# Lumina-Group/libzkp

Measured on AMD Instinct MI355X. Metric: proofs/sec (whole node) + ms/proof p50, 4096-proof mixed batch (range / equality / membership / improvement) per MI355X, higher is better.
Workload: dtype u32/u64 integer limbs (10x25.5-bit GF(2^255-19), BN254 Fq on 9x29-bit limbs in the MSM loops and 10x26-bit elsewhere, 8x32-bit Fr and scalars mod l, 2x64-bit f128)

## Files before the change

### libzkp_amd/csrc/bp_steps.h

```cpp
#pragma once
#include "fe25519.h"
#include "sc25519.h"
#include "ge25519.h"
#include "keccak.h"

namespace zkp {

constexpr uint32_t BP_N = 64;
constexpr uint32_t BASE_B = 0, BASE_BB = 1, BASE_G = 2, BASE_H = 66, NBASE = 130;
constexpr uint32_t WBITS = 10, NWIN = 26, NENT = 512, DIGW = 13, NWIN_U64 = 7, NIELS_W = 30, SUBTAB_W = NENT * NIELS_W;
constexpr uint32_t TAPE_SLOTS = 132;
constexpr uint32_t P1_V = 0, P1_A = 2, P1_NSLOTS = 260;
constexpr uint32_t P2_NSLOTS = 4;
constexpr uint32_t PR_NSLOTS = 130;
ZKP_HD constexpr uint32_t p1_s(uint32_t n) { return 3 + 2 * n; }
ZKP_HD constexpr uint32_t tape_slots(uint32_t n) { return 2 * n + 4; }
ZKP_HD constexpr uint32_t rp_bytes(uint32_t lg) { return 32 * (9 + 2 * lg); }
constexpr uint32_t GE_W = 40;
enum { SC_Y = 0, SC_Z, SC_X, SC_W, SC_U, SC_UINV, SC_T0, SC_T1, SC_T2, SC_NUM };
enum { KIND_RANGE_MIN = 0, KIND_RANGE_MAX, KIND_THRESHOLD, KIND_CONSISTENCY, KIND_BULLETPROOF, KIND_NUM };

struct BpView {
    uint32_t M;
    uint32_t n, lg;
// ... 102 lines not shown
    n = ge_niels_select(d < 0, ge_niels_neg(n), n);
    return ge_madd(acc, n);
}
ZKP_HD inline void st_ge(uint32_t* p, uint32_t idx, uint32_t row, uint32_t rows, const ge& g) {
    uint32_t* q = p + (size_t)idx * GE_W * rows + row;
    ZKP_UNROLL for (int k = 0; k < 10; k++) {
        q[(size_t)k * rows] = g.X.v[k]; q[(size_t)(10 + k) * rows] = g.Y.v[k];
        q[(size_t)(20 + k) * rows] = g.Z.v[k]; q[(size_t)(30 + k) * rows] = g.T.v[k];
    }
}
ZKP_HD inline ge ld_ge(const uint32_t* p, uint32_t idx, uint32_t row, uint32_t rows) {
    ge g; const uint32_t* q = p + (size_t)idx * GE_W * rows + row;
    ZKP_UNROLL for (int k = 0; k < 10; k++) {
        g.X.v[k] = q[(size_t)k * rows]; g.Y.v[k] = q[(size_t)(10 + k) * rows];
        g.Z.v[k] = q[(size_t)(20 + k) * rows]; g.T.v[k] = q[(size_t)(30 + k) * rows];
    }
    return g;
}
struct MsmView {
    uint32_t rows, nslots, nchunks;
    const uint32_t* table;
    const uint32_t* digits;
    const uint16_t* slot_base;
    const uint16_t* slot_scalar;
    const uint8_t* slot_nwin;
    const uint16_t* chunk_begin;
    const uint16_t* chunk_win0;
    const uint16_t* chunk_nwin;
    uint32_t* partial;
    const uint32_t* acc_init;
    uint32_t nwin = 0, nent = 0, digw = 0;
    uint32_t slot_ent = 0, uneven = 0;
    const uint32_t* steps = nullptr; const uint32_t* chunk_step0 = nullptr;
};
ZKP_HD inline void msm_chunk_ref(const MsmView& m, uint32_t chunk, uint32_t row) {
    ge acc = ge_identity();
    uint32_t s = m.chunk_begin[chunk], w = m.chunk_win0[chunk];
    for (uint32_t left = m.chunk_nwin[chunk]; left > 0; left--) {
        const uint32_t srow = m.slot_scalar ? m.slot_scalar[s] : s;
        const int32_t d = ld_digit(m.digits, srow, w, row, m.rows);
        if (d != 0) acc = msm_accumulate_digit(acc, d, m.table + ((size_t)m.slot_base[s] * NWIN + w) * SUBTAB_W);
        if (++w == m.slot_nwin[s]) { s++; w = 0; }
    }
    st_ge(m.partial, chunk, row, m.rows, acc);
}
struct ReduceView {
    uint32_t rows, ntargets;
    const uint32_t* partial;
    const uint16_t* target_chunk_begin;
    uint32_t* enc;
    const uint64_t* out_off;
    uint8_t* out;
    const uint32_t* corr;
};
ZKP_HD inline void reduce_encode_thread(const ReduceView& r, uint32_t target, uint32_t row) {
    const uint32_t c0 = r.target_chunk_begin[target], c1 = r.target_chunk_begin[target + 1];
    ge acc = ld_ge(r.partial, c0, row, r.rows);
    for (uint32_t c = c0 + 1; c < c1; c++) acc = ge_add(acc, ld_ge(r.partial, c, row, r.rows));
    sc e; ge_ristretto_encode(e.v, acc);
    st_sc(r.enc, target, row, r.rows, e);
    if (r.out_off != nullptr && target == 0) put_bytes(r.out + r.out_off[row], e.v, 8);
}

ZKP_HD inline void strobe_save(const BpView& V, uint32_t job, const Strobe& s) {
    for (int i = 0; i < 50; i++) V.tstate[(size_t)i * V.M + job] = s.base[i * s.stride];
    V.tstate[(size_t)50 * V.M + job] = s.pos; V.tstate[(size_t)51 * V.M + job] = s.pos_begin;
}
ZKP_HD inline void strobe_load(const BpView& V, uint32_t job, Strobe& s) {
    for (int i = 0; i < 50; i++) s.base[i * s.stride] = V.tstate[(size_t)i * V.M + job];
    s.pos = V.tstate[(size_t)50 * V.M + job]; s.pos_begin = V.tstate[(size_t)51 * V.M + job];
}
ZKP_HD inline sc merlin_challenge_scalar(Strobe& s, const char* label, uint32_t label_len) {
    uint32_t w[16]; merlin_challenge_words(s, label, label_len, w, 16);
    return sc_from_wide(w);
}
ZKP_HD inline void merlin_append_scalar(Strobe& s, const char* label, uint32_t label_len, const sc& raw) { merlin_append_words(s, label, label_len, raw.v, 8); }

ZKP_HD inline void step_transcript1(const BpView& V, uint32_t job, Strobe& s) {
    const uint32_t M = V.M;
    switch (V.kind[job]) {
        case KIND_RANGE_MIN: merlin_init(s, "libzkp_range_min", 16); break;
        case KIND_RANGE_MAX: merlin_init(s, "libzkp_range_max", 16); break;
        case KIND_THRESHOLD: merlin_init(s, "libzkp_threshold", 16); break;
        case KIND_CONSISTENCY: merlin_init(s, "libzkp_consistency", 18); break;
        default: merlin_init(s, "libzkp_bulletproof", 18); break;
    }
    merlin_append_bytes(s, "dom-sep", 7, "rangeproof v1", 13);
    merlin_append_u64(s, "n", 1, V.n);
    merlin_append_u64(s, "m", 1, 1);
    const sc Ve = ld_sc(V.enc, 0, job, M), Ae = ld_sc(V.enc, 1, job, M), Se = ld_sc(V.enc, 2, job, M);
    merlin_append_words(s, "V", 1, Ve.v, 8);
    merlin_append_words(s, "A", 1, Ae.v, 8);
    merlin_append_words(s, "S", 1, Se.v, 8);
    const sc y = merlin_challenge_scalar(s, "y", 1);
    const sc z = merlin_challenge_scalar(s, "z", 1);
    strobe_save(V, job, s);
    st_sc(V.scal, SC_Y, job, M, y);
    st_sc(V.scal, SC_Z, job, M, z);
    const sc yinv = sc_invert(y);
    for (uint32_t h = 0; h < 2; h++) {
        const sc base = h ? yinv : y;
        sc p = sc_one();
        for (uint32_t b = 0; b < 8; b++) { st_sc(V.ypq, 16 * h + b, job, M, p); p = sc_mul(p, base); }
        sc q = sc_one();
        for (uint32_t a = 0; a < 8; a++) { st_sc(V.ypq, 16 * h + 8 + a, job, M, q); q = sc_mul(q, p); }
    }
    uint8_t* pr = V.out + V.proof_off[job];
    put_bytes(pr, Ae.v, 8); put_bytes(pr + 32, Se.v, 8);
    put_bytes(V.out + V.commit_off[job], Ve.v, 8);
// ... 199 lines not shown
```

### libzkp_amd/csrc/g16_impl.inc

```

namespace {

struct G16Key {
    bool loaded = false;
    uint32_t n_inst = 0, n_wit = 0, nv = 0, n_rows = 0, m = 0, logm = 0;
    G16Circuit C{};
    std::vector<void*> allocs;
    uint32_t *table_g1 = nullptr, *table_g2 = nullptr;
    G16Radix rx = g16_radix(G16_WBITS_DEFAULT);
    int shared_tables = -1;
    uint64_t table_bytes = 0;
    struct Chunking { DevLayout lay; const uint32_t* corr = nullptr; const uint16_t* scal = nullptr; };
    std::vector<SlotList> targets_g1, targets_g2;
    std::vector<uint16_t> hscal_g1, hscal_g2;
    std::map<uint64_t, Chunking> lays_g1, lays_g2;
    uint64_t win_g1 = 0, win_g2 = 0;
    const uint32_t *init_g1 = nullptr, *init_g2 = nullptr;
    G16Vk vk{}; bool vk_ready = false;
    uint64_t vk_table_bytes = 0;
    bool verifier_only() const { return vk_ready && !loaded; }
    const uint32_t *vm_kconst = nullptr, *vm_lines = nullptr;
};
struct G16Run {
    void* buf = nullptr; size_t cap = 0; hipStream_t side = nullptr, side2 = nullptr; hipEvent_t ev[4] = {nullptr, nullptr, nullptr, nullptr};
// ... 37 lines not shown
g2_aff host_g2_generator() {
    static const char* dec[4] = {"10857046999023057135944570762232829481370756359578518086990519993285655852781",
                                 "11559732032986387107991004021392285783925812861821192530917403151452391805634",
                                 "8495653923123431417604973247489272438418190587263600148770280649306958101930",
                                 "4082367875863433681332203403145435568316851327593401208105741076214120093531"};
    fq c[4];
    for (int k = 0; k < 4; k++) {
        fq acc = fq_zero(); const fq ten = fq_from_u64(10);
        for (const char* q = dec[k]; *q; q++) acc = fq_add(fq_mul(acc, ten), fq_from_u64((uint64_t)(*q - '0')));
        c[k] = acc;
    }
    return g2_aff{fq2{c[0], c[1]}, fq2{c[2], c[3]}};
}
g1_aff host_g1_generator() { return g1_aff{fq_from_u64(1), fq_from_u64(2)}; }
struct MsmOffsets { g1_jac o1; g2_jac o2; bool ready = false; };
MsmOffsets g_off;
std::once_flag g_off_once;
void compute_offsets();
void ensure_offsets() { std::call_once(g_off_once, compute_offsets); }
void compute_offsets() {
    uint8_t h[32]; const char* tag = "libzkp-amd msm offset"; sha256_host(h, (const uint8_t*)tag, strlen(tag));
    uint32_t k[8]; memcpy(k, h, 32); k[7] &= 0x0fffffffu;
    g_off.o1 = jac_mul_raw(jac_from_aff(host_g1_generator()), k);
    g_off.o2 = jac_mul_raw(jac_from_aff(host_g2_generator()), k);
    g_off.ready = true;
}
template <class J> J host_neg_multiple(const J& o, uint32_t k) {
    J acc = o; for (uint32_t i = 1; i < k; i++) acc = jac_add(acc, o);
    return jac_neg(acc);
}
template <class J> void append_words(std::vector<uint32_t>& v, const J& p) { const uint32_t* w = reinterpret_cast<const uint32_t*>(&p); for (size_t i = 0; i < sizeof(J) / 4; i++) v.push_back(w[i]); }
int upload_offset_point(G16Key& K, bool g2, const uint32_t** d_init) {
    ensure_offsets();
    std::vector<uint32_t> init;
    if (!g2) append_words(init, g_off.o1); else append_words(init, g_off.o2);
    return dev_upload(K, d_init, init);
}
uint32_t choose_chunks(uint64_t windows, uint32_t ntargets, uint32_t rows, uint32_t resident, uint32_t tb) {
    const uint32_t groups = (rows + tb - 1) / tb;
    uint32_t hi = (uint32_t)(windows / 8); if (hi > 2048) hi = 2048; if (hi < ntargets) hi = ntargets;
    uint32_t best = ntargets; double best_cost = 1e300;
    for (uint32_t c = ntargets; c <= hi; c++) {
        const double rounds = std::ceil((double)c * groups / resident);
        const double cost = rounds * (std::ceil((double)windows / c) + 2.5) + 0.25 * c / 8.0;
        if (cost < best_cost) { best_cost = cost; best = c; }
    }
    return best;
}
enum { G16_PART_ALL = 0, G16_PART_AB = 1, G16_PART_C = 2 };
int get_chunking(G16Key& K, bool g2, int part, uint32_t rows, const G16Key::Chunking** out) {
    const uint32_t resident = (uint32_t)dev().num_cu * g16_msm_blocks_per_cu(g2);
    const auto& all = g2 ? K.targets_g2 : K.targets_g1;
    std::vector<SlotList> targets;
    if (part == G16_PART_ALL) targets = all;
    else if (part == G16_PART_AB) targets.assign(all.begin(), all.begin() + 2);
    else targets.assign(all.begin() + 2, all.end());
    uint64_t windows = 0; for (auto& t : targets) for (auto& sl : t) windows += sl.second;
    uint32_t c = choose_chunks(windows, (uint32_t)targets.size(), rows, resident, g16_msm_rows_per_block(g2));
    if (g_budget_request >= 10000) c = g_budget_request - 10000;
    auto& cache = g2 ? K.lays_g2 : K.lays_g1;
    const uint64_t key = (uint64_t)part << 32 | c;
    auto it = cache.find(key);
    if (it == cache.end()) {
        const MsmLayout L = make_layout_even(targets, c);
        G16Key::Chunking ch; int rc;
        const auto& hs = g2 ? K.hscal_g2 : K.hscal_g1;
        std::vector<uint16_t> scal; for (uint16_t b : L.slot_base) scal.push_back(hs[b]);
        const GatherShape shape{K.rx.nent, K.rx.slot_ent, K.rx.uneven ? 1u : 0u, K.rx.digw};
        if ((rc = upload_layout(ch.lay, L, &shape, scal.data()))) return rc;
        std::vector<uint32_t> corr;
        for (uint32_t t = 0; t < L.ntargets(); t++) {
            const uint32_t k = L.target_chunk_begin[t + 1] - L.target_chunk_begin[t];
            if (!g2) append_words(corr, host_neg_multiple(g_off.o1, k)); else append_words(corr, host_neg_multiple(g_off.o2, k));
        }
        if ((rc = dev_upload(K, &ch.corr, corr))) return rc;
        if ((rc = dev_upload(K, &ch.scal, scal))) return rc;
        it = cache.emplace(key, ch).first;
    }
    *out = &it->second;
    return 0;
}


uint64_t key_table_bytes(size_t n1, size_t n2, uint32_t wbits, bool uneven = false) {
    const G16Radix rx = g16_radix(wbits, uneven);
    return ((uint64_t)n1 * g16_table_entry_words(false, true) + (uint64_t)n2 * g16_table_entry_words(true, true)) * 4ull * rx.slot_ent;
}
int choose_radix(size_t n1, size_t n2, uint32_t* wbits_out, bool* uneven_out) {
    *uneven_out = false;
    const int forced = env_int("ZKP_HIP_G16_WBITS", 0);
    if (forced) {
        if (forced < (int)G16_WBITS_MIN || forced > (int)G16_WBITS_MAX) return fail(ZKP_HIP_E_ARGUMENT, "ZKP_HIP_G16_WBITS must be 8..15");
        *wbits_out = (uint32_t)forced; *uneven_out = forced == 14 && env_int("ZKP_HIP_G16_UNEVEN", 1) != 0; return 0;
    }
    size_t free_b = 0, total_b = 0;
    HIP_TRY(hipMemGetInfo(&free_b, &total_b));
    const int budget_mb = env_int("ZKP_HIP_G16_TABLE_BUDGET_MB", 0);
    const uint64_t reserve = 8ull << 30;
    const uint64_t fits = free_b > reserve ? (uint64_t)((free_b - reserve) * 0.45) : 0;
    uint64_t budget = budget_mb > 0 ? (uint64_t)budget_mb << 20 : fits;
    uint32_t first = G16_WBITS_KNEE;
    if (budget_mb > 0) {
        first = G16_WBITS_DEFAULT;
        if (G16_WBITS_DEFAULT == 14 && env_int("ZKP_HIP_G16_UNEVEN", 1) != 0 && key_table_bytes(n1, n2, 14, true) <= budget) { *wbits_out = 14; *uneven_out = true; return 0; }
    }
    for (uint32_t w = first; w >= G16_WBITS_MIN; w--)
        if (key_table_bytes(n1, n2, w) <= budget) { *wbits_out = w; return 0; }
    char msg[256];
    snprintf(msg, sizeof msg, "not enough device memory for the proving key's window tables: %llu MB at the smallest radix (2^%u), budget %llu MB (%llu MB free)",
             (unsigned long long)(key_table_bytes(n1, n2, G16_WBITS_MIN) >> 20), G16_WBITS_MIN, (unsigned long long)(budget >> 20), (unsigned long long)(free_b >> 20));
    return fail(ZKP_HIP_E_RUNTIME, msg);
}
struct SharedTables { int hip_dev, kind; uint8_t digest[32]; uint32_t wbits; uint32_t *g1, *g2; int refs; };
struct TableRegistry { std::mutex mu; std::vector<SharedTables> v; std::map<int, std::unique_ptr<std::mutex>> build_mu; };
TableRegistry& table_registry() { static TableRegistry* r = new TableRegistry(); return *r; }
void release_shared_tables(G16Key& K) {
    if (K.shared_tables < 0) return;
    TableRegistry& R = table_registry();
    std::lock_guard<std::mutex> lk(R.mu);
    SharedTables& e = R.v[(size_t)K.shared_tables];
    if (--e.refs == 0) { (void)hipFree(e.g1); (void)hipFree(e.g2); e.g1 = e.g2 = nullptr; }
    K.shared_tables = -1; K.table_g1 = K.table_g2 = nullptr;
}

template <uint32_t AW, class Pt>
int build_tables(G16Key& K, const std::vector<Pt>& bases, uint32_t** table, bool msm_form, const G16Radix& rx, bool owned = true) {
    std::vector<uint32_t> flat; flat.reserve(bases.size() * AW);
    for (auto& b : bases) { const uint32_t* w = reinterpret_cast<const uint32_t*>(&b); for (uint32_t k = 0; k < AW; k++) flat.push_back(w[k]); }
    uint32_t* d_bases = nullptr; int rc;
    if ((rc = dev_upload(K, &d_bases, flat))) return rc;
    const size_t words = bases.size() * (size_t)rx.slot_ent * g16_table_entry_words(AW == 40, msm_form);
    uint32_t* tab = nullptr;
    if (hipMalloc(&tab, words * 4 + 64) != hipSuccess) {
        (void)hipGetLastError();
        char msg[200]; snprintf(msg, sizeof msg, "out of device memory allocating %llu MB of key tables (radix 2^%u)", (unsigned long long)((words * 4) >> 20), rx.wbits);
        return fail(ZKP_HIP_E_RUNTIME, msg);
    }
    if (owned) K.allocs.push_back(tab);
    g16_launch_build_table(AW == 40, d_bases, (uint32_t)bases.size(), tab, dev().stream, msm_form, rx);
    HIP_TRY(hipGetLastError());
    HIP_TRY(hipStreamSynchronize(dev().stream));
    *table = tab;
    return 0;
}

void release_key(G16Key& K) {
    (void)hipDeviceSynchronize();
    release_shared_tables(K);
    for (void* p : K.allocs) (void)hipFree(p);
    for (auto& e : K.lays_g1) free_layout(e.second.lay);
    for (auto& e : K.lays_g2) free_layout(e.second.lay);
    K = G16Key();
}
int load_key_body(int kind, const uint8_t* pk, uint64_t len);
int no_proving_key(const G16Key& K) {
    return fail(ZKP_HIP_E_ARGUMENT, K.verifier_only() ? "only a verifying key is loaded for this circuit: proving needs the proving key (zkp_hip_groth16_load_key)"
                                                      : "no proving key loaded for this circuit (zkp_hip_groth16_load_key)");
}
int load_key_locked(int kind, const uint8_t* pk, uint64_t len) {
    if (kind != G16_EQUALITY && kind != G16_MEMBERSHIP) return fail(ZKP_HIP_E_ARGUMENT, "unknown circuit kind");
    G16Key& K = g16s().key[kind];
    if (K.loaded || K.shared_tables >= 0 || !K.allocs.empty()) release_key(K);
    int rc;
    try { rc = load_key_body(kind, pk, len); }
    catch (...) { release_key(K); throw; }
    if (rc) { const std::string keep = t_err; release_key(K); t_err = keep; }
// ... 2 lines not shown
int install_verifying_key(G16Key& K, const G16VkBlob& B) {
    int rc;
    K.vk_ready = false;
    std::vector<uint32_t> icw; for (auto& e : B.abc) append_words(icw, e.p);
    append_words(icw, B.alpha_g1.p);
    const uint32_t* d_ic = nullptr;
    if ((rc = dev_upload(K, &d_ic, icw))) return rc;
    std::vector<g1_aff> ic_pts; for (auto& e : B.abc) ic_pts.push_back(e.p);
    ic_pts.push_back(B.alpha_g1.p);
    uint32_t* d_ic_tab = nullptr;
    const G16Radix vrx = g16_radix(G16V_WBITS);
    if ((rc = build_tables<20>(K, ic_pts, &d_ic_tab, false, vrx))) return rc;
    K.vk_table_bytes = (uint64_t)ic_pts.size() * vrx.slot_ent * g16_table_entry_words(false, false) * 4ull;
    K.vk.gamma = B.gamma_g2.p; K.vk.delta = B.delta_g2.p; K.vk.beta = B.beta_g2.p; K.vk.n_ic = (uint32_t)B.abc.size(); K.vk.ic = d_ic; K.vk.ic_table = d_ic_tab;
    K.vk.ml_alpha_beta = miller_loop(B.beta_g2.p, aff_neg(B.alpha_g1.p));
    std::vector<uint32_t> kc(6 * 20), lines;
    g16_vm_key_constants(B.beta_g2.p, aff_neg(B.alpha_g1.p), B.gamma_g2.p, B.delta_g2.p, kc.data(), lines);
    if ((rc = dev_upload(K, &K.vm_kconst, kc)) || (rc = dev_upload(K, &K.vm_lines, lines))) return rc;
    K.vk_ready = true;
    return 0;
}
int ensure_mimc_dev() {
    if (g16s().mimc_dev) return 0;
    ensure_mimc_constants();
    std::vector<uint32_t> mc; for (auto& c : g_mimc_host) put_fr(mc, c);
    HIP_TRY(hipMalloc(&g16s().mimc_dev, mc.size() * 4)); HIP_TRY(hipMemcpy(g16s().mimc_dev, mc.data(), mc.size() * 4, hipMemcpyHostToDevice));
    return 0;
}
int load_key_body(int kind, const uint8_t* pk, uint64_t len) {
    G16Key& K = g16s().key[kind];
    const HostR1CS cs = kind == G16_EQUALITY ? build_equality_r1cs() : build_membership_r1cs();
    int rc;
    KeyReader R{pk, len};
    G16VkBlob B;
    const int format = g16_read_key_prefix(R, B);
    if (format == G16_BLOB_MALFORMED)
        return fail(ZKP_HIP_E_ARGUMENT, "malformed proving key or verifying key (expected ark-serialize uncompressed ProvingKey<Bn254>, or its VerifyingKey<Bn254> alone)");
    if (format == G16_BLOB_VERIFYING_KEY) {
        if (const char* why = g16_check_verifying_key(B, cs.n_inst)) return fail(ZKP_HIP_E_ARGUMENT, why);
        return install_verifying_key(K, B);
    }
    if ((rc = upload_circuit(K, cs)) || (rc = ensure_mimc_dev())) return rc;
    const G1Pt &alpha_g1 = B.alpha_g1; const G2Pt &beta_g2 = B.beta_g2, &delta_g2 = B.delta_g2;
    const std::vector<G1Pt>& abc = B.abc;
    G1Pt beta_g1, delta_g1;
    std::vector<G1Pt> aq, b1q, hq, lq; std::vector<G2Pt> b2q;
    if (parse_g1(R, beta_g1.inf, beta_g1.p) || parse_g1(R, delta_g1.inf, delta_g1.p) ||
        parse_vec_g1(R, aq) || parse_vec_g1(R, b1q) || parse_vec_g2(R, b2q) || parse_vec_g1(R, hq) || parse_vec_g1(R, lq) || !R.ok || R.left != 0)
        return fail(ZKP_HIP_E_ARGUMENT, "malformed proving key (expected ark-serialize uncompressed ProvingKey<Bn254>)");
    if (aq.size() != K.nv || b1q.size() != K.nv || b2q.size() != K.nv || hq.size() != K.m - 1 || lq.size() != K.n_wit || abc.size() != K.n_inst)
        return fail(ZKP_HIP_E_ARGUMENT, "proving key does not match the circuit shape");
    if (alpha_g1.inf || beta_g1.inf || delta_g1.inf || beta_g2.inf || delta_g2.inf) return fail(ZKP_HIP_E_ARGUMENT, "degenerate proving key");
    const uint32_t SC_H = K.nv, SC_R = K.nv + K.m - 1, SC_S = SC_R + 1, SC_NRS = SC_R + 2, SC_ONE = SC_R + 3;
    uint8_t digest[32]; sha256_host(digest, pk, len);
    TableRegistry& TR = table_registry();
    std::mutex* bm = nullptr;
    { std::lock_guard<std::mutex> lk(TR.mu); auto& up = TR.build_mu[dev().hip_dev]; if (!up) up.reset(new std::mutex()); bm = up.get(); }
    std::lock_guard<std::mutex> build_lock(*bm);
    {
        const bool forced = env_int("ZKP_HIP_G16_WBITS", 0) != 0;
        uint32_t wb = 0; bool uneven = false; int found = -1;
        {
            std::lock_guard<std::mutex> lk(TR.mu);
            for (size_t i = 0; i < TR.v.size() && !forced; i++)
                if (TR.v[i].refs > 0 && TR.v[i].hip_dev == dev().hip_dev && TR.v[i].kind == kind && !memcmp(TR.v[i].digest, digest, 32)) {
                    found = (int)i; TR.v[i].refs++; wb = TR.v[i].wbits & 0xffu; uneven = (TR.v[i].wbits >> 8) != 0;
                    K.shared_tables = found; K.table_g1 = TR.v[i].g1; K.table_g2 = TR.v[i].g2;
                    break;
                }
        }
        if (found < 0 && (rc = choose_radix(aq.size() + b1q.size() + lq.size() + hq.size() + 5, b2q.size() + 2, &wb, &uneven))) return rc;
        K.rx = g16_radix(wb, uneven);
    }
    const uint32_t NWIN = K.rx.nwin;
    auto var_nwin = [&](uint32_t k) -> uint8_t { return g16_class_nwin(k < cs.n_inst ? cs.inst_nwin[k] : cs.wit_nwin[k - cs.n_inst], K.rx); };
    std::vector<g1_aff> bases1; std::vector<g2_aff> bases2;
    std::vector<uint16_t> scal1, scal2;
    std::vector<SlotList> t1(3), t2(1);
    auto add1 = [&](int target, const G1Pt& pt, uint32_t scal, uint8_t nwin) {
        if (pt.inf) return;
        t1[target].push_back({(uint16_t)bases1.size(), nwin}); bases1.push_back(pt.p); scal1.push_back((uint16_t)scal);
    };
    auto add2 = [&](const G2Pt& pt, uint32_t scal, uint8_t nwin) {
        if (pt.inf) return;
        t2[0].push_back({(uint16_t)bases2.size(), nwin}); bases2.push_back(pt.p); scal2.push_back((uint16_t)scal);
    };
    if (K.nv + K.m + 3 > 65535 || 3ull * K.nv + K.m + 8 > 65535) return fail(ZKP_HIP_E_UNSUPPORTED, "circuit too large for 16-bit slot indices");
    for (uint32_t k = 0; k < K.nv; k++) add1(0, aq[k], k, var_nwin(k));
    add1(0, delta_g1, SC_R, NWIN); add1(0, alpha_g1, SC_ONE, 1);
    for (uint32_t k = 0; k < K.nv; k++) add1(1, b1q[k], k, var_nwin(k));
    add1(1, delta_g1, SC_S, NWIN); add1(1, beta_g1, SC_ONE, 1);
    for (uint32_t k = 0; k < K.n_wit; k++) add1(2, lq[k], K.n_inst + k, var_nwin(K.n_inst + k));
    for (uint32_t i = 0; i + 1 < K.m; i++) add1(2, hq[i], SC_H + i, NWIN);
    add1(2, delta_g1, SC_NRS, NWIN);
    for (uint32_t k = 0; k < K.nv; k++) add2(b2q[k], k, var_nwin(k));
    add2(delta_g2, SC_S, NWIN); add2(beta_g2, SC_ONE, 1);
    {
        std::vector<g1_aff> ob; std::vector<uint16_t> os;
        for (auto& t : t1) for (auto& sl : t) { ob.push_back(bases1[sl.first]); os.push_back(scal1[sl.first]); }
        uint16_t idx = 0; for (auto& t : t1) for (auto& sl : t) sl.first = idx++;
        bases1.swap(ob); scal1.swap(os);
    }
    K.targets_g1 = t1; K.targets_g2 = t2;
    for (auto& t : t1) for (auto& sl : t) K.win_g1 += sl.second;
    for (auto& t : t2) for (auto& sl : t) K.win_g2 += sl.second;
    K.hscal_g1 = scal1; K.hscal_g2 = scal2;
    if ((rc = upload_offset_point(K, false, &K.init_g1)) || (rc = upload_offset_point(K, true, &K.init_g2))) return rc;
    if (K.shared_tables < 0) {
        TableRegistry& R = TR;
        int found = -1;
        {
            std::lock_guard<std::mutex> lk(R.mu);
            for (size_t i = 0; i < R.v.size(); i++)
                if (R.v[i].refs > 0 && R.v[i].hip_dev == dev().hip_dev && R.v[i].kind == kind && R.v[i].wbits == (K.rx.wbits | K.rx.uneven << 8) && !memcmp(R.v[i].digest, digest, 32)) { found = (int)i; R.v[i].refs++; break; }
        }
        if (found < 0) {
            uint32_t *t1 = nullptr, *t2 = nullptr;
            if ((rc = build_tables<20>(K, bases1, &t1, true, K.rx, false))) return rc;
            if ((rc = build_tables<40>(K, bases2, &t2, true, K.rx, false))) { (void)hipFree(t1); return rc; }
            std::lock_guard<std::mutex> lk(R.mu);
            SharedTables e{}; e.hip_dev = dev().hip_dev; e.kind = kind; memcpy(e.digest, digest, 32); e.wbits = K.rx.wbits | K.rx.uneven << 8; e.g1 = t1; e.g2 = t2; e.refs = 1;
            R.v.push_back(e); found = (int)R.v.size() - 1;
        }
        std::lock_guard<std::mutex> lk(R.mu);
        K.shared_tables = found; K.table_g1 = R.v[(size_t)found].g1; K.table_g2 = R.v[(size_t)found].g2;
    }
    K.table_bytes = key_table_bytes(bases1.size(), bases2.size(), K.rx.wbits, K.rx.uneven);
    K.vk_ready = false;
    if (!g16_check_verifying_key(B, K.n_inst) && (rc = install_verifying_key(K, B))) return rc;
    K.loaded = true;
    return 0;
}


fr tape_fr(const uint32_t seed[8], uint32_t idx, uint32_t slot) { uint32_t w[16]; tape_draw64(w, seed, idx, slot); return fp_from_wide<FrParams>(w); }

int gpu_scalar_mults(bool g2, const std::vector<fr>& scalars, std::vector<uint8_t>& out_bytes) {
    const uint32_t rows = (uint32_t)scalars.size(), AW = g2 ? 40 : 20, JW = g2 ? G2_JAC_W : G1_JAC_W, PB = g2 ? 128 : 64;
    std::vector<uint32_t> base;
    if (!g2) append_words(base, host_g1_generator()); else append_words(base, host_g2_generator());
    ensure_offsets();
    std::vector<uint32_t> offs;
    if (!g2) { append_words(offs, g_off.o1); append_words(offs, jac_neg(g_off.o1)); } else { append_words(offs, g_off.o2); append_words(offs, jac_neg(g_off.o2)); }
    const G16Radix rx = g16_radix(10);
    std::vector<uint32_t> dig((size_t)rx.digw * rows);
    for (uint32_t i = 0; i < rows; i++) {
        sc raw; fp_to_raw(raw.v, scalars[i]); uint32_t pk[G16_DIGW_MAX]; g16_recode(pk, raw, rx);
        for (uint32_t k = 0; k < rx.digw; k++) dig[(size_t)k * rows + i] = pk[k];
    }
    uint32_t *d_base = nullptr, *d_tab = nullptr, *d_dig = nullptr, *d_part = nullptr, *d_offs = nullptr, *d_sums = nullptr; uint8_t* d_out = nullptr;
    uint16_t* d_meta = nullptr; uint8_t* d_nwin = nullptr; uint32_t* d_steps = nullptr;
    DevScope mem;
    HIP_TRY(mem.alloc(&d_base, AW * 4)); HIP_TRY(mem.alloc(&d_tab, (size_t)rx.slot_ent * g16_table_entry_words(g2, true) * 4 + 64)); HIP_TRY(mem.alloc(&d_dig, dig.size() * 4));
    HIP_TRY(mem.alloc(&d_part, (size_t)JW * 4 * rows)); HIP_TRY(mem.alloc(&d_sums, (size_t)JW * 4 * rows)); HIP_TRY(mem.alloc(&d_offs, offs.size() * 4));
    HIP_TRY(hipMemcpy(d_offs, offs.data(), offs.size() * 4, hipMemcpyHostToDevice)); HIP_TRY(mem.alloc(&d_out, (size_t)PB * rows)); HIP_TRY(mem.alloc(&d_meta, 32)); HIP_TRY(mem.alloc(&d_nwin, 16));
    const uint16_t meta[7] = {0, 0, 0, 0, (uint16_t)rx.nwin, 0, 1};
    const uint8_t nwin = (uint8_t)rx.nwin;
    HIP_TRY(hipMemcpy(d_base, base.data(), AW * 4, hipMemcpyHostToDevice));
    HIP_TRY(hipMemcpy(d_dig, dig.data(), dig.size() * 4, hipMemcpyHostToDevice));
    HIP_TRY(hipMemcpy(d_meta, meta, 14, hipMemcpyHostToDevice)); HIP_TRY(hipMemcpy(d_nwin, &nwin, 1, hipMemcpyHostToDevice));
    uint32_t steps_words = 0;
    {
        MsmLayout L1; L1.slot_base = {0}; L1.slot_nwin = {(uint8_t)rx.nwin}; L1.chunk_begin = {0}; L1.chunk_win0 = {0}; L1.chunk_nwin = {(uint16_t)rx.nwin}; L1.target_chunk_begin = {0, 1};
        std::vector<uint32_t> steps, step0;
        const GatherShape shape{rx.nent, rx.slot_ent, rx.uneven ? 1u : 0u, rx.digw};
        if (!make_gather_steps(L1, nullptr, shape, steps, step0)) return fail(ZKP_HIP_E_UNSUPPORTED, "window tables of more than 2^32 entries");
        steps.insert(steps.end(), step0.begin(), step0.end());
        HIP_TRY(mem.alloc(&d_steps, steps.size() * 4));
        HIP_TRY(hipMemcpy(d_steps, steps.data(), steps.size() * 4, hipMemcpyHostToDevice));
        steps_words = (uint32_t)(steps.size() - step0.size());
    }
    g16_launch_build_table(g2, d_base, 1, d_tab, dev().stream, true, rx);
    MsmView m; m.nwin = rx.nwin; m.nent = rx.nent; m.digw = rx.digw; m.slot_ent = rx.slot_ent; m.uneven = rx.uneven; m.rows = rows; m.nslots = 1; m.nchunks = 1; m.table = d_tab; m.digits = d_dig;
    m.slot_base = d_meta; m.slot_scalar = d_meta + 1; m.slot_nwin = d_nwin; m.chunk_begin = d_meta + 2; m.chunk_win0 = d_meta + 3; m.chunk_nwin = d_meta + 4; m.partial = d_part; m.acc_init = d_offs;
// ... 82 lines not shown

int run_g16(int kind, uint32_t rows, const uint64_t* d_value, const uint64_t* d_set_vals, const uint32_t* d_set_len, const uint8_t* d_seeds,
            uint8_t* d_out, uint64_t stride, hipStream_t st, uint32_t lane = 0) {
    G16Key& K = g16s().key[kind];
    if (!K.loaded) return no_proving_key(K);
    const uint32_t nsc = g16_nscalars(K.nv, K.m);
    const G16Key::Chunking *c1 = nullptr, *c1c = nullptr, *c2 = nullptr;
    int rc;
    if ((rc = get_chunking(K, false, G16_PART_AB, rows, &c1)) || (rc = get_chunking(K, true, G16_PART_ALL, rows, &c2))) return rc;
    if ((rc = get_chunking(K, false, G16_PART_C, rows, &c1c))) return rc;
    size_t off = 0;
    auto sz = [&](size_t bytes) { size_t o = off; off += align_up(bytes); return o; };
    const size_t W = (size_t)32 * rows;
    const size_t o_z = sz(W * K.nv), o_sd = sz((size_t)K.rx.digw * 4 * rows * nsc), o_rs = sz(W * 2), o_p1 = sz((size_t)c1->lay.nchunks * G1_JAC_W * 4 * rows),
                 o_p1c = sz((size_t)c1c->lay.nchunks * G1_JAC_W * 4 * rows), o_p2 = sz((size_t)c2->lay.nchunks * G2_JAC_W * 4 * rows),
                 o_s1 = sz((size_t)3 * G1_JAC_W * 4 * rows), o_s2 = sz((size_t)G2_JAC_W * 4 * rows), o_t1 = sz((size_t)G16_CPARTS * G1_JAC_W * 4 * rows),
                 o_qe = sz((size_t)2 * 9 * K.m * 4 * rows);
    G16Run& RW = g16s().run[kind][lane & 1u];
    if (off > RW.cap) {
        if (RW.buf) { HIP_TRY(hipDeviceSynchronize()); HIP_TRY(hipFree(RW.buf)); RW.buf = nullptr; RW.cap = 0; }
        HIP_TRY(hipMalloc(&RW.buf, off)); RW.cap = off;
    }
    uint8_t* base = (uint8_t*)RW.buf;
    G16View V{}; V.rx = K.rx; V.rows = rows; V.kind = (uint32_t)kind; V.n_inst = K.n_inst; V.n_wit = K.n_wit; V.nv = K.nv; V.m = K.m;
    V.value = d_value; V.set_vals = d_set_vals; V.set_len = d_set_len; V.seeds = reinterpret_cast<const uint32_t*>(d_seeds); V.mimc_c = g16s().mimc_dev;
    V.z = (uint32_t*)(base + o_z); V.sdig = (uint32_t*)(base + o_sd); V.rs = (uint32_t*)(base + o_rs); V.out = d_out; V.stride = stride;
    V.qap_evals = (uint32_t*)(base + o_qe);
    uint32_t *p1 = (uint32_t*)(base + o_p1), *p1c = (uint32_t*)(base + o_p1c), *p2 = (uint32_t*)(base + o_p2), *s1 = (uint32_t*)(base + o_s1), *s2 = (uint32_t*)(base + o_s2), *t1 = (uint32_t*)(base + o_t1);
    if (!RW.last) {
        for (auto& e : RW.ev) HIP_TRY(hipEventCreateWithFlags(&e, hipEventDisableTiming));
        HIP_TRY(hipEventCreateWithFlags(&RW.last, hipEventDisableTiming));
    }
    G16Run& R0 = g16s().run[kind][0];
    if (!R0.side) {
        static const int side_level = env_int("ZKP_HIP_G16_SIDE_PRIORITY", 2), side2_level = env_int("ZKP_HIP_G16_SIDE2_PRIORITY", 0);
        HIP_TRY(hipStreamCreateWithPriority(&R0.side, hipStreamNonBlocking, stream_priority(side_level)));
        HIP_TRY(hipStreamCreateWithPriority(&R0.side2, hipStreamNonBlocking, stream_priority(side2_level)));
    }
    hipStream_t const side = R0.side, side2 = R0.side2;
    hipEvent_t ev_wit = RW.ev[0], ev_ab = RW.ev[1], ev_c = RW.ev[2], ev_cp = RW.ev[3];
    ReduceView R2{}; R2.rows = rows; R2.ntargets = 1; R2.partial = p2; R2.target_chunk_begin = c2->lay.target_chunk_begin; R2.corr = c2->corr;
    if (RW.used) HIP_TRY(hipStreamWaitEvent(st, RW.last, 0));
    ZKP_TRACED("k_g16_witness", st, g16_launch_witness(V, st));
    ZKP_TRACED("k_g16_zdigits", st, g16_launch_zdigits(V, st));
    HIP_TRY(hipEventRecord(ev_wit, st));
    HIP_TRY(hipStreamWaitEvent(side, ev_wit, 0));
    { TraceMark tm_("k_g16_qap", side); HIP_TRY(g16_launch_qap(V, K.C, side)); }
    if ((rc = launch_msm_key(false, K.rx, *c1c, K.table_g1, K.init_g1, rows, V.sdig, p1c, side))) return rc;
    ReduceView Rc{}; Rc.rows = rows; Rc.ntargets = 1; Rc.partial = p1c; Rc.target_chunk_begin = c1c->lay.target_chunk_begin; Rc.corr = c1c->corr;
    ZKP_TRACED("k_sum_t<G1Msm>", side, g16_launch_sum(false, Rc, s1 + (size_t)2 * G1_JAC_W * rows, side));
    HIP_TRY(hipEventRecord(ev_c, side));
    if ((rc = launch_msm_key(false, K.rx, *c1, K.table_g1, K.init_g1, rows, V.sdig, p1, st))) return rc;
    ReduceView Rab{}; Rab.rows = rows; Rab.ntargets = 2; Rab.partial = p1; Rab.target_chunk_begin = c1->lay.target_chunk_begin; Rab.corr = c1->corr;
    HIP_TRY(hipEventRecord(ev_ab, st));
    HIP_TRY(hipStreamWaitEvent(side2, ev_ab, 0));
    ZKP_TRACED("k_sum_t<G1Msm>", side2, g16_launch_sum(false, Rab, s1, side2));
    ZKP_TRACED("k_g16_cparts", side2, g16_launch_cparts(V, s1, t1, side2));
    HIP_TRY(hipEventRecord(ev_cp, side2));
    if ((rc = launch_msm_key(true, K.rx, *c2, K.table_g2, K.init_g2, rows, V.sdig, p2, st))) return rc;
    ZKP_TRACED("k_sum_t<G2Msm>", st, g16_launch_sum(true, R2, s2, st));
    HIP_TRY(hipStreamWaitEvent(st, ev_c, 0));
    HIP_TRY(hipStreamWaitEvent(st, ev_cp, 0));
    ZKP_TRACED("k_g16_final", st, g16_launch_final(V, s1, s2, t1, st));
    HIP_TRY(hipGetLastError());
    HIP_TRY(hipEventRecord(RW.last, st)); RW.used = true;
    return 0;
}

int prove_g16_host(int kind, uint64_t n, const uint64_t* values, const uint64_t* sets_flat, const uint32_t* set_counts, const std::vector<uint8_t>& valid,
                   const uint8_t* seeds, uint8_t* out, uint64_t stride, uint32_t* out_len, int32_t* status) {
    if (g16s().key[kind].verifier_only()) return no_proving_key(g16s().key[kind]);
    std::vector<uint64_t> v, sv; std::vector<uint32_t> sl, idx; std::vector<uint8_t> sd;
    size_t pos = 0; int any = 0;
    memset(out, 0, stride * n);
    for (uint64_t i = 0; i < n; i++) {
        const uint32_t cnt = set_counts ? set_counts[i] : 0;
        if (valid[i]) {
            idx.push_back((uint32_t)i); v.push_back(values[i]);
            sd.insert(sd.end(), seeds + 32 * i, seeds + 32 * i + 32);
            if (kind == G16_MEMBERSHIP) { sl.push_back(cnt); for (uint32_t k = 0; k < G16_MAX_SET; k++) sv.push_back(k < cnt ? sets_flat[pos + k] : 0); }
            const uint32_t plen = kind == G16_EQUALITY ? 298u : 10u + 4u + 8u * cnt + 256u + 32u;
            if (plen > stride) return fail(ZKP_HIP_E_ARGUMENT, "stride too small for the proof envelope");
            out_len[i] = plen; status[i] = ZKP_HIP_OK;
        } else { out_len[i] = 0; status[i] = ZKP_HIP_INVALID_INPUT; any = 1; }
        pos += cnt;
    }
    const uint32_t rows = (uint32_t)idx.size();
    if (rows == 0) return any;
    hipStream_t st = dev().stream;
    uint64_t *d_v = nullptr, *d_sv = nullptr; uint32_t* d_sl = nullptr; uint8_t *d_sd = nullptr, *d_out = nullptr;
    DevScope mem;
    HIP_TRY(mem.alloc(&d_v, 8ull * rows)); HIP_TRY(mem.alloc(&d_sd, 32ull * rows)); HIP_TRY(mem.alloc(&d_out, stride * rows));
    HIP_TRY(hipMemcpyAsync(d_v, v.data(), 8ull * rows, hipMemcpyHostToDevice, st));
    HIP_TRY(hipMemcpyAsync(d_sd, sd.data(), 32ull * rows, hipMemcpyHostToDevice, st));
    HIP_TRY(hipMemsetAsync(d_out, 0, stride * rows, st));
    if (kind == G16_MEMBERSHIP) {
        HIP_TRY(mem.alloc(&d_sv, 8ull * sv.size())); HIP_TRY(mem.alloc(&d_sl, 4ull * rows));
        HIP_TRY(hipMemcpyAsync(d_sv, sv.data(), 8ull * sv.size(), hipMemcpyHostToDevice, st));
        HIP_TRY(hipMemcpyAsync(d_sl, sl.data(), 4ull * rows, hipMemcpyHostToDevice, st));
    }
    int rc = run_g16(kind, rows, d_v, d_sv, d_sl, d_sd, d_out, stride, st);
    std::vector<uint8_t> tmp;
    if (rc == 0) {
        tmp.resize(stride * rows);
        HIP_TRY(hipMemcpyAsync(tmp.data(), d_out, stride * rows, hipMemcpyDeviceToHost, st));
        HIP_TRY(hipStreamSynchronize(st));
// ... 274 lines not shown
```

### libzkp_amd/csrc/msm_kernel.h

```cpp
#pragma once
#include <hip/hip_runtime.h>
#include "bp_steps.h"

using namespace zkp;
static constexpr int TW = 64;
static constexpr int TB = 256;


template <class T> constexpr size_t gather_lds_bytes() { return T::GATHER_PREFETCH < 0 ? (size_t)4 * 2 * (T::GATHER_W / 4) * 64 * 16 : 0; }
template <class T>
__global__ void __launch_bounds__(256, T::GATHER_WAVES) k_msm_gather(MsmView m, uint32_t ngroups, uint32_t nblocks) {
    constexpr uint32_t V4 = T::GATHER_W / 4;
    constexpr uint32_t SV4 = T::GATHER_STRIDE / 4;
    const uint32_t tid = threadIdx.x;
    const uint32_t per_xcd = (nblocks + 7) / 8;
    const uint32_t linear = (blockIdx.x & 7u) * per_xcd + (blockIdx.x >> 3);
    if (linear >= nblocks) return;
    const uint32_t chunk = linear / ngroups, group = linear % ngroups;
    const uint32_t row = group * 256u + tid;
    const bool active = row < m.rows;
    const uint32_t st0 = m.chunk_step0[chunk], left = m.chunk_step0[chunk + 1] - st0;
    const uint2* const steps = reinterpret_cast<const uint2*>(m.steps) + st0;
    typename T::GAcc acc = T::to_gather(m.acc_init ? T::load(m.acc_init, 0, 0, 1) : T::identity());
    const uint4* const table4 = reinterpret_cast<const uint4*>(m.table);
// ... 14 lines not shown
        int32_t d = T::digit(digit_word(steps[0]), steps[0].y & 1u);
        uint32_t q0 = left > 1 ? digit_word(steps[1]) : 0u, q1 = left > 2 ? digit_word(steps[2]) : 0u;
        dma(0, steps[0], d);
        for (uint32_t i = 0; i < left; i++) {
            int32_t dn = 0;
            asm volatile("s_waitcnt vmcnt(0)" ::: "memory");
            uint4 e[V4];
            if (d != 0) { ZKP_UNROLL for (uint32_t k = 0; k < V4; k++) e[k] = wbuf[(cb * V4 + k) * 64u + lane]; }
            if (i + 1 < left) { const uint2 ds = steps[i + 1]; dn = T::digit(q0, ds.y & 1u); dma(cb ^ 1u, ds, dn); }
            const uint32_t qn = i + 3 < left ? digit_word(steps[i + 3]) : 0u;
            if (d != 0) acc = T::accumulate_entry(acc, d, reinterpret_cast<const uint32_t*>(e));
            cb ^= 1u; d = dn; q0 = q1; q1 = qn;
        }
        if (active) T::store(m.partial, chunk, row, m.rows, T::from_gather(acc));
        return;
#endif
    } else {
        constexpr int LEAD = T::GATHER_PREFETCH;
        uint4 e[LEAD + 1][V4]; int32_t dd[LEAD + 1];
        auto fetch = [&](uint4* dst, const uint2 ds, int32_t d) {
            if (d == 0) return;
            const uint4* src = entry_of(ds, d);
            ZKP_UNROLL for (uint32_t k = 0; k < V4; k++) dst[k] = src[k];
        };
        uint32_t qpre[LEAD + 2];
        ZKP_UNROLL for (int k = 0; k < LEAD + 2; k++) qpre[k] = (uint32_t)k < left ? digit_word(steps[k]) : 0u;
        ZKP_UNROLL for (int k = 0; k < LEAD; k++) {
            dd[k] = 0;
            if ((uint32_t)k < left) { const uint2 ds = steps[k]; dd[k] = T::digit(qpre[k], ds.y & 1u); fetch(e[k], ds, dd[k]); }
        }
        uint32_t q0 = qpre[LEAD], q1 = qpre[LEAD + 1];
        if constexpr (T::GATHER_PRIO > 0) __builtin_amdgcn_s_setprio(T::GATHER_PRIO);
        for (uint32_t i = 0; i < left; i++) {
            dd[LEAD] = 0;
            if (i + LEAD < left) { const uint2 ds = steps[i + LEAD]; dd[LEAD] = T::digit(q0, ds.y & 1u); fetch(e[LEAD], ds, dd[LEAD]); }
            const uint32_t qn = i + LEAD + 2 < left ? digit_word(steps[i + LEAD + 2]) : 0u;
            if (dd[0] != 0) acc = T::accumulate_entry(acc, dd[0], reinterpret_cast<const uint32_t*>(e[0]));
            ZKP_UNROLL for (int k = 0; k < LEAD; k++) { ZKP_UNROLL for (uint32_t v = 0; v < V4; v++) e[k][v] = e[k + 1][v]; dd[k] = dd[k + 1]; }
            q0 = q1; q1 = qn;
        }
    }
    if (active) T::store(m.partial, chunk, row, m.rows, T::from_gather(acc));
}

template <class T, uint32_t ROWS, uint32_t NTHREADS, uint32_t MIN_WAVES = 1>
__global__ void __launch_bounds__(NTHREADS, MIN_WAVES) k_sum_t(ReduceView R, uint32_t* sums) {
    ZKP_RAISE_PRIO();
    constexpr uint32_t SLICES = NTHREADS / ROWS;
    static_assert(NTHREADS % ROWS == 0 && (SLICES & (SLICES - 1)) == 0, "slices per row: a power of two");
    __shared__ uint32_t lds[T::ACC_W * (NTHREADS / 2)];
    const uint32_t rl = threadIdx.x % ROWS, slice = threadIdx.x / ROWS;
    const uint32_t row = blockIdx.x * ROWS + rl, target = blockIdx.y;
    const bool active = row < R.rows;
    const uint32_t c0 = R.target_chunk_begin[target], c1 = R.target_chunk_begin[target + 1];
    typename T::Acc acc = T::identity();
    bool have = false;
    if (active) {
        for (uint32_t c = c0 + slice; c < c1; c += SLICES) {
            const typename T::Acc p = T::load(R.partial, c, row, R.rows);
            acc = have ? T::add(acc, p) : p;
            have = true;
        }
    }
    for (uint32_t stride = SLICES / 2; stride >= 1; stride >>= 1) {
        if (slice >= stride && slice < 2 * stride) T::store(lds, 0, (slice - stride) * ROWS + rl, NTHREADS / 2, acc);
        __syncthreads();
        if (slice < stride) acc = T::add(acc, T::load(lds, 0, slice * ROWS + rl, NTHREADS / 2));
        __syncthreads();
    }
    if (slice == 0 && active) {
        if (R.corr) acc = T::add(acc, T::load(R.corr, target, 0, 1));
        T::store(sums, target, row, R.rows, acc);
    }
}
```

### libzkp_amd/csrc/zkp_hip.hip

```cpp
#include <hip/hip_runtime.h>
#include <mutex>
#include <memory>
#include <algorithm>
#include <map>
#include <array>
#include <type_traits>
#include <atomic>
#include <thread>
#include <condition_variable>
#include <functional>
#include <deque>
#include <new>
#include <exception>
#include <cstring>
#include <string>
#include <vector>
#include <cstdio>
#include <cstdlib>
#include <cmath>
#include <chrono>
#include <sys/random.h>
#include "bp_layout.h"
#include "g16_steps.h"
#include "sha256_host.h"
#include "g16_circuit.h"
#include "g16_keyblob.h"
#include "msm_kernel.h"
#include "g16_launch.h"
#include "g16_verify_launch.h"
#include "stark_launch.h"
#include "bpv_launch.h"
#include "edg_launch.h"
#include "batch_self_check.h"
#include "../../include/libzkp_hip.h"


__global__ void __launch_bounds__(TB) k_build_range(JobBuf J, uint32_t n, const uint64_t* value, const uint64_t* mn, const uint64_t* mx, uint32_t lg,
                                                    uint8_t* out, uint64_t stride, uint32_t* out_len, int32_t* status) {
    ZKP_RAISE_PRIO();
    const uint32_t op = blockIdx.x * TB + threadIdx.x;
    if (op < n) step_build_range(J, op, value, mn, mx, lg, out, stride, out_len, status);
}
__global__ void __launch_bounds__(TB) k_ctask(CtView T) {
    ZKP_RAISE_PRIO();
    const uint32_t c = blockIdx.x * TB + threadIdx.x;
    if (c < T.C) step_ctask(T, c);
}
__global__ void __launch_bounds__(TB) k_tape(BpView V) {
    ZKP_RAISE_PRIO();
    const uint32_t job = blockIdx.x * TB + threadIdx.x;
    if (job < V.M) step_tape(V, blockIdx.y, job);
}
static constexpr uint32_t LAT_WAVES = 5;
__global__ void __launch_bounds__(TB, LAT_WAVES) k_poly(BpView V) {
    ZKP_RAISE_PRIO();
    const uint32_t job = blockIdx.x * TB + threadIdx.x;
    if (job < V.M) step_poly(V, blockIdx.y, job);
}
__device__ __forceinline__ ScTriple triple_tree8(ScTriple t, uint32_t* lds) {
    const uint32_t lane = threadIdx.x, grp = lane >> 3;
    for (uint32_t stride = 4; stride >= 1; stride >>= 1) {
        if (grp >= stride && grp < 2 * stride) {
            ZKP_UNROLL for (int k = 0; k < 8; k++) { lds[k * TW + lane] = t.a.v[k]; lds[(8 + k) * TW + lane] = t.b.v[k]; lds[(16 + k) * TW + lane] = t.c.v[k]; }
        }
        __syncthreads();
        if (grp < stride) {
            ScTriple o; const uint32_t src = lane + stride * 8;
            ZKP_UNROLL for (int k = 0; k < 8; k++) { o.a.v[k] = lds[k * TW + src]; o.b.v[k] = lds[(8 + k) * TW + src]; o.c.v[k] = lds[(16 + k) * TW + src]; }
            t = triple_add(t, o);
        }
        __syncthreads();
    }
    return t;
}
__global__ void __launch_bounds__(TW, LAT_WAVES) k_poly_sum(BpView V) {
    ZKP_RAISE_PRIO();
    __shared__ uint32_t lds[24 * TW];
    const uint32_t job = blockIdx.x * 8 + (threadIdx.x & 7u), part = threadIdx.x >> 3;
    const bool active = job < V.M;
// ... 1150 lines not shown
```

Baseline: 338,300.

## Share Groth16 A/B1 G1 MSM bases via overlapping reduction chunk ranges

When a proving-key point in the A query equals the matching point in the B1 query, that slot is moved into a separate shared target instead of being added to both the A and B MSMs. The reduction step now takes an optional per-target chunk end, so A sums the chunks for [A-only, shared] and B sums [shared, B-only]. Correction offsets and table sizing are adjusted to match. The aim is to cut duplicated windowed-MSM gathers and table memory; the benefit depends on how often the two queries hold identical points. It also changes the table cache key and the target layout for the C part.

```diff
diff --git a/libzkp_amd/csrc/bp_steps.h b/libzkp_amd/csrc/bp_steps.h
--- a/libzkp_amd/csrc/bp_steps.h
+++ b/libzkp_amd/csrc/bp_steps.h
@@ -178,9 +178,11 @@
     const uint64_t* out_off;
     uint8_t* out;
     const uint32_t* corr;
+    const uint16_t* target_chunk_end = nullptr;
 };
+ZKP_HD inline uint32_t reduce_chunk_end(const ReduceView& r, uint32_t target) { return r.target_chunk_end ? r.target_chunk_end[target] : r.target_chunk_begin[target + 1]; }
 ZKP_HD inline void reduce_encode_thread(const ReduceView& r, uint32_t target, uint32_t row) {
-    const uint32_t c0 = r.target_chunk_begin[target], c1 = r.target_chunk_begin[target + 1];
+    const uint32_t c0 = r.target_chunk_begin[target], c1 = reduce_chunk_end(r, target);
     ge acc = ld_ge(r.partial, c0, row, r.rows);
     for (uint32_t c = c0 + 1; c < c1; c++) acc = ge_add(acc, ld_ge(r.partial, c, row, r.rows));
     sc e; ge_ristretto_encode(e.v, acc);
diff --git a/libzkp_amd/csrc/g16_impl.inc b/libzkp_amd/csrc/g16_impl.inc
--- a/libzkp_amd/csrc/g16_impl.inc
+++ b/libzkp_amd/csrc/g16_impl.inc
@@ -113,9 +113,9 @@
     const uint32_t resident = (uint32_t)dev().num_cu * g16_msm_blocks_per_cu(g2);
     const auto& all = g2 ? K.targets_g2 : K.targets_g1;
     std::vector<SlotList> targets;
-    if (part == G16_PART_ALL) targets = all;
-    else if (part == G16_PART_AB) targets.assign(all.begin(), all.begin() + 2);
-    else targets.assign(all.begin() + 2, all.end());
+    if (part == G16_PART_ALL) { if (!g2) return fail(ZKP_HIP_E_ARGUMENT, "G16_PART_ALL is the G2 launch"); targets = all; }
+    else if (part == G16_PART_AB) targets = g16_ab_targets(all[0], all[1], all[2]);
+    else targets.assign(all.begin() + 3, all.end());
     uint64_t windows = 0; for (auto& t : targets) for (auto& sl : t) windows += sl.second;
     uint32_t c = choose_chunks(windows, (uint32_t)targets.size(), rows, resident, g16_msm_rows_per_block(g2));
     if (g_budget_request >= 10000) c = g_budget_request - 10000;
@@ -130,8 +130,10 @@
         const GatherShape shape{K.rx.nent, K.rx.slot_ent, K.rx.uneven ? 1u : 0u, K.rx.digw};
         if ((rc = upload_layout(ch.lay, L, &shape, scal.data()))) return rc;
         std::vector<uint32_t> corr;
-        for (uint32_t t = 0; t < L.ntargets(); t++) {
-            const uint32_t k = L.target_chunk_begin[t + 1] - L.target_chunk_begin[t];
+        const bool ab3 = part == G16_PART_AB && L.ntargets() == 3;
+        const G16AbRanges ab = ab3 ? g16_ab_ranges(L) : G16AbRanges{};
+        for (uint32_t t = 0; t < (ab3 ? 2u : L.ntargets()); t++) {
+            const uint32_t k = ab3 ? ab.end[t] - ab.begin[t] : L.target_chunk_begin[t + 1] - L.target_chunk_begin[t];
             if (!g2) append_words(corr, host_neg_multiple(g_off.o1, k)); else append_words(corr, host_neg_multiple(g_off.o2, k));
         }
         if ((rc = dev_upload(K, &ch.corr, corr))) return rc;
@@ -172,7 +174,7 @@
              (unsigned long long)(key_table_bytes(n1, n2, G16_WBITS_MIN) >> 20), G16_WBITS_MIN, (unsigned long long)(budget >> 20), (unsigned long long)(free_b >> 20));
     return fail(ZKP_HIP_E_RUNTIME, msg);
 }
-struct SharedTables { int hip_dev, kind; uint8_t digest[32]; uint32_t wbits; uint32_t *g1, *g2; int refs; };
+struct SharedTables { int hip_dev, kind; uint8_t digest[32]; uint32_t wbits; bool share_ab; uint32_t *g1, *g2; int refs; };
 struct TableRegistry { std::mutex mu; std::vector<SharedTables> v; std::map<int, std::unique_ptr<std::mutex>> build_mu; };
 TableRegistry& table_registry() { static TableRegistry* r = new TableRegistry(); return *r; }
 void release_shared_tables(G16Key& K) {
@@ -281,6 +283,9 @@
         return fail(ZKP_HIP_E_ARGUMENT, "proving key does not match the circuit shape");
     if (alpha_g1.inf || beta_g1.inf || delta_g1.inf || beta_g2.inf || delta_g2.inf) return fail(ZKP_HIP_E_ARGUMENT, "degenerate proving key");
     const uint32_t SC_H = K.nv, SC_R = K.nv + K.m - 1, SC_S = SC_R + 1, SC_NRS = SC_R + 2, SC_ONE = SC_R + 3;
+    const bool share_ab = env_int("ZKP_HIP_G16_SHARE_AB", 1) != 0;
+    std::vector<uint8_t> var_class(cs.inst_nwin); var_class.insert(var_class.end(), cs.wit_nwin.begin(), cs.wit_nwin.end());
+    const G16AbSlots ab = g16_ab_slots(aq, b1q, var_class, share_ab);
     uint8_t digest[32]; sha256_host(digest, pk, len);
     TableRegistry& TR = table_registry();
     std::mutex* bm = nullptr;
@@ -292,20 +297,20 @@
         {
             std::lock_guard<std::mutex> lk(TR.mu);
             for (size_t i = 0; i < TR.v.size() && !forced; i++)
-                if (TR.v[i].refs > 0 && TR.v[i].hip_dev == dev().hip_dev && TR.v[i].kind == kind && !memcmp(TR.v[i].digest, digest, 32)) {
+                if (TR.v[i].refs > 0 && TR.v[i].hip_dev == dev().hip_dev && TR.v[i].kind == kind && TR.v[i].share_ab == share_ab && !memcmp(TR.v[i].digest, digest, 32)) {
                     found = (int)i; TR.v[i].refs++; wb = TR.v[i].wbits & 0xffu; uneven = (TR.v[i].wbits >> 8) != 0;
                     K.shared_tables = found; K.table_g1 = TR.v[i].g1; K.table_g2 = TR.v[i].g2;
                     break;
                 }
         }
-        if (found < 0 && (rc = choose_radix(aq.size() + b1q.size() + lq.size() + hq.size() + 5, b2q.size() + 2, &wb, &uneven))) return rc;
+        if (found < 0 && (rc = choose_radix(aq.size() + b1q.size() - ab.s.size() + lq.size() + hq.size() + 5, b2q.size() + 2, &wb, &uneven))) return rc;
         K.rx = g16_radix(wb, uneven);
     }
     const uint32_t NWIN = K.rx.nwin;
     auto var_nwin = [&](uint32_t k) -> uint8_t { return g16_class_nwin(k < cs.n_inst ? cs.inst_nwin[k] : cs.wit_nwin[k - cs.n_inst], K.rx); };
     std::vector<g1_aff> bases1; std::vector<g2_aff> bases2;
     std::vector<uint16_t> scal1, scal2;
-    std::vector<SlotList> t1(3), t2(1);
+    std::vector<SlotList> t1(4), t2(1);
     auto add1 = [&](int target, const G1Pt& pt, uint32_t scal, uint8_t nwin) {
         if (pt.inf) return;
         t1[target].push_back({(uint16_t)bases1.size(), nwin}); bases1.push_back(pt.p); scal1.push_back((uint16_t)scal);
@@ -315,13 +320,14 @@
         t2[0].push_back({(uint16_t)bases2.size(), nwin}); bases2.push_back(pt.p); scal2.push_back((uint16_t)scal);
     };
     if (K.nv + K.m + 3 > 65535 || 3ull * K.nv + K.m + 8 > 65535) return fail(ZKP_HIP_E_UNSUPPORTED, "circuit too large for 16-bit slot indices");
-    for (uint32_t k = 0; k < K.nv; k++) add1(0, aq[k], k, var_nwin(k));
+    for (auto& sl : ab.a) add1(0, aq[sl.first], sl.first, var_nwin(sl.first));
     add1(0, delta_g1, SC_R, NWIN); add1(0, alpha_g1, SC_ONE, 1);
-    for (uint32_t k = 0; k < K.nv; k++) add1(1, b1q[k], k, var_nwin(k));
-    add1(1, delta_g1, SC_S, NWIN); add1(1, beta_g1, SC_ONE, 1);
-    for (uint32_t k = 0; k < K.n_wit; k++) add1(2, lq[k], K.n_inst + k, var_nwin(K.n_inst + k));
-    for (uint32_t i = 0; i + 1 < K.m; i++) add1(2, hq[i], SC_H + i, NWIN);
-    add1(2, delta_g1, SC_NRS, NWIN);
+    for (auto& sl : ab.s) add1(1, aq[sl.first], sl.first, var_nwin(sl.first));
+    for (auto& sl : ab.b) add1(2, b1q[sl.first], sl.first, var_nwin(sl.first));
+    add1(2, delta_g1, SC_S, NWIN); add1(2, beta_g1, SC_ONE, 1);
+    for (uint32_t k = 0; k < K.n_wit; k++) add1(3, lq[k], K.n_inst + k, var_nwin(K.n_inst + k));
+    for (uint32_t i = 0; i + 1 < K.m; i++) add1(3, hq[i], SC_H + i, NWIN);
+    add1(3, delta_g1, SC_NRS, NWIN);
     for (uint32_t k = 0; k < K.nv; k++) add2(b2q[k], k, var_nwin(k));
     add2(delta_g2, SC_S, NWIN); add2(beta_g2, SC_ONE, 1);
     {
@@ -341,14 +347,14 @@
         {
             std::lock_guard<std::mutex> lk(R.mu);
             for (size_t i = 0; i < R.v.size(); i++)
-                if (R.v[i].refs > 0 && R.v[i].hip_dev == dev().hip_dev && R.v[i].kind == kind && R.v[i].wbits == (K.rx.wbits | K.rx.uneven << 8) && !memcmp(R.v[i].digest, digest, 32)) { found = (int)i; R.v[i].refs++; break; }
+                if (R.v[i].refs > 0 && R.v[i].hip_dev == dev().hip_dev && R.v[i].kind == kind && R.v[i].wbits == (K.rx.wbits | K.rx.uneven << 8) && R.v[i].share_ab == share_ab && !memcmp(R.v[i].digest, digest, 32)) { found = (int)i; R.v[i].refs++; break; }
         }
         if (found < 0) {
             uint32_t *t1 = nullptr, *t2 = nullptr;
             if ((rc = build_tables<20>(K, bases1, &t1, true, K.rx, false))) return rc;
             if ((rc = build_tables<40>(K, bases2, &t2, true, K.rx, false))) { (void)hipFree(t1); return rc; }
             std::lock_guard<std::mutex> lk(R.mu);
-            SharedTables e{}; e.hip_dev = dev().hip_dev; e.kind = kind; memcpy(e.digest, digest, 32); e.wbits = K.rx.wbits | K.rx.uneven << 8; e.g1 = t1; e.g2 = t2; e.refs = 1;
+            SharedTables e{}; e.hip_dev = dev().hip_dev; e.kind = kind; memcpy(e.digest, digest, 32); e.wbits = K.rx.wbits | K.rx.uneven << 8; e.share_ab = share_ab; e.g1 = t1; e.g2 = t2; e.refs = 1;
             R.v.push_back(e); found = (int)R.v.size() - 1;
         }
         std::lock_guard<std::mutex> lk(R.mu);
@@ -537,6 +543,7 @@
     HIP_TRY(hipEventRecord(ev_c, side));
     if ((rc = launch_msm_key(false, K.rx, *c1, K.table_g1, K.init_g1, rows, V.sdig, p1, st))) return rc;
     ReduceView Rab{}; Rab.rows = rows; Rab.ntargets = 2; Rab.partial = p1; Rab.target_chunk_begin = c1->lay.target_chunk_begin; Rab.corr = c1->corr;
+    if (c1->lay.ntargets == 3) Rab.target_chunk_end = c1->lay.target_chunk_begin + 2;
     HIP_TRY(hipEventRecord(ev_ab, st));
     HIP_TRY(hipStreamWaitEvent(side2, ev_ab, 0));
     ZKP_TRACED("k_sum_t<G1Msm>", side2, g16_launch_sum(false, Rab, s1, side2));
diff --git a/libzkp_amd/csrc/g16_share.h b/libzkp_amd/csrc/g16_share.h
--- /dev/null
+++ b/libzkp_amd/csrc/g16_share.h
@@ -0,0 +1,38 @@
+#pragma once
+#include <cstdint>
+#include <vector>
+#include "bp_layout.h"
+#include "g16_keyblob.h"
+
+namespace zkp {
+
+inline bool g16_shared_point(const G1Pt& a, const G1Pt& b) { return !a.inf && !b.inf && fq_eq(a.p.x, b.p.x) && fq_eq(a.p.y, b.p.y); }
+
+struct G16AbSlots { SlotList a, s, b; };
+inline G16AbSlots g16_ab_slots(const std::vector<G1Pt>& aq, const std::vector<G1Pt>& b1q, const std::vector<uint8_t>& cls, bool share) {
+    G16AbSlots out;
+    const size_t n = aq.size() < b1q.size() ? aq.size() : b1q.size();
+    for (size_t k = 0; k < aq.size(); k++) {
+        if (aq[k].inf) continue;
+        if (share && k < n && g16_shared_point(aq[k], b1q[k])) out.s.push_back({(uint16_t)k, cls[k]});
+        else out.a.push_back({(uint16_t)k, cls[k]});
+    }
+    for (size_t k = 0; k < b1q.size(); k++) {
+        if (b1q[k].inf || (share && k < n && g16_shared_point(aq[k], b1q[k]))) continue;
+        out.b.push_back({(uint16_t)k, cls[k]});
+    }
+    return out;
+}
+
+inline std::vector<SlotList> g16_ab_targets(const SlotList& a, const SlotList& s, const SlotList& b) {
+    if (s.empty()) return {a, b};
+    return {a, s, b};
+}
+struct G16AbRanges { uint16_t begin[2], end[2]; };
+inline G16AbRanges g16_ab_ranges(const MsmLayout& L) {
+    const auto& t = L.target_chunk_begin;
+    if (L.ntargets() == 3) return {{t[0], t[1]}, {t[2], t[3]}};
+    return {{t[0], t[1]}, {t[1], t[2]}};
+}
+
+}
diff --git a/libzkp_amd/csrc/msm_kernel.h b/libzkp_amd/csrc/msm_kernel.h
--- a/libzkp_amd/csrc/msm_kernel.h
+++ b/libzkp_amd/csrc/msm_kernel.h
@@ -90,7 +90,7 @@
     const uint32_t rl = threadIdx.x % ROWS, slice = threadIdx.x / ROWS;
     const uint32_t row = blockIdx.x * ROWS + rl, target = blockIdx.y;
     const bool active = row < R.rows;
-    const uint32_t c0 = R.target_chunk_begin[target], c1 = R.target_chunk_begin[target + 1];
+    const uint32_t c0 = R.target_chunk_begin[target], c1 = reduce_chunk_end(R, target);
     typename T::Acc acc = T::identity();
     bool have = false;
     if (active) {
diff --git a/libzkp_amd/csrc/zkp_hip.hip b/libzkp_amd/csrc/zkp_hip.hip
--- a/libzkp_amd/csrc/zkp_hip.hip
+++ b/libzkp_amd/csrc/zkp_hip.hip
@@ -25,6 +25,7 @@
 #include "sha256_host.h"
 #include "g16_circuit.h"
 #include "g16_keyblob.h"
+#include "g16_share.h"
 #include "msm_kernel.h"
 #include "g16_launch.h"
 #include "g16_verify_launch.h"
```

After: 349,000, median of 6. +3.2%, better.
